# omuses/hqp

Hardware: AMD Instinct MI355X
Metric: KKT factor+solve/sec (fp64) (higher is better)
Workload: dtype f64; 1 GPU; C4 = BASELINE configs[3], the metric's 10^6-variable DOCP: multistage LQ optimal control QP, K=200 stages, nx=5000 states, nu=50 controls -> n=1015000 me=1005000 m=20000, dense fx/fu handed over as blocks, x_0 fixed, box bounds on u; plugin LQDOCP (STAGED engine), one system per GPU; stages=200, nx=5000, nu=50, n=1015000, me=1005000, m=20000, plugin=LQDOCP, kkt_dim_full=2040000

## Files before the change

__graft_entry__.py:

```python
from __future__ import annotations

import os
import subprocess
import sys

ROOT = os.path.dirname(os.path.abspath(__file__))
if ROOT not in sys.path:
    sys.path.insert(0, ROOT)

CSRC = os.path.join(ROOT, "hqp_amd", "csrc")
LIB = os.path.join(ROOT, "hqp_amd", "libhqpkkt.so")
LIB_RCCL = os.path.join(ROOT, "hqp_amd", "libhqpkkt_rccl.so")
HIPCC = os.environ.get("HIPCC", "/opt/rocm/bin/hipcc")


def _stale(target, sources):
    if not os.path.exists(target):
        return True
    t = os.path.getmtime(target)
    return any(os.path.getmtime(s) > t for s in sources)


def build(force=False):
    units = ("hqpkkt.hip", "tree.hip", "staged_engine.hip", "ip_loops.hip", "analysis.cpp", "staged_plan.cpp")
    srcs = [os.path.join(CSRC, f) for f in units + ("hqpkkt_handle.hpp", "device_common.hip.h", "analysis.hpp", "kernels.hip.h",
                                                    "ipdriver.hip.h", "factor_blk.hip.h", "solve_top.hip.h", "staged.hip.h", "staged_gemm.hip.h", "staged_sparse.hip.h", "staged_profile.hip.h", "staged_rows.hip.h",
                                                    "staged_host.hip.h", "staged_plan.hpp", "sk_table.hpp", "gemm_form.hpp")]
    srcs.append(os.path.join(ROOT, "include", "hqpkkt.h"))
    if force or _stale(LIB, srcs):
        cmd = [HIPCC, "--offload-arch=gfx950", "-O3", "-std=c++17", "-fPIC", "-shared",
               "-Wall", "-Wno-unused-function", "-o", LIB] + [os.path.join(CSRC, f) for f in units]
        subprocess.check_call(cmd, cwd=ROOT)
    rsrc = [os.path.join(CSRC, "rccl_exchange.cpp"), os.path.join(ROOT, "include", "hqpkkt_rccl.h")]
    if force or _stale(LIB_RCCL, rsrc):
        subprocess.check_call([HIPCC, "--offload-arch=gfx950", "-O2", "-std=c++17", "-fPIC", "-shared", "-Wall",
                               "-o", LIB_RCCL, rsrc[0], "-ldl"], cwd=ROOT)
    subprocess.check_call(["make", "-s", "-C", os.path.join(ROOT, "oracle"), "all"])
    import hqp_amd
    from hqp_amd import _lib
    L = _lib.lib()
    for sym in _lib.SYMBOLS:
# ... 50 lines not shown
```

hqp_amd/_lib.py:

```python
from __future__ import annotations

import ctypes as C
import os

import numpy as np

_HERE = os.path.dirname(os.path.abspath(__file__))
LIB_PATH = os.environ.get("HQPKKT_LIB") or os.path.join(_HERE, "libhqpkkt.so")

OK, E_SIZES, E_MEM, E_SING, E_FORMAT, E_NULL, E_RANGE, E_INTERN, E_DEVICE = 0, 1, 3, 4, 6, 8, 10, 17, 100
MODE_FULL, MODE_REDUCED, MODE_STAGED = 0, 1, 2
LOC_HOST, LOC_DEVICE = 0, 1
DYN_DENSE, DYN_SPARSE, DYN_PROFILE = 0, 1, 3

SYMBOLS = [
    "hqpkkt_default_opts", "hqpkkt_create", "hqpkkt_destroy", "hqpkkt_analyze",
    "hqpkkt_set_values", "hqpkkt_factor", "hqpkkt_step", "hqpkkt_residual", "hqpkkt_solve",
    "hqpkkt_get_sbw", "hqpkkt_get_perm", "hqpkkt_set_tol", "hqpkkt_set_eps",
    "hqpkkt_set_stream", "hqpkkt_get_stats", "hqpkkt_strerror", "hqpkkt_debug_get",
    "hqpkkt_selftest_mfma", "hqpkkt_set_profile", "hqpkkt_get_profile",
    "hqpkkt_profile_class_name", "hqpkkt_set_shard", "hqpkkt_debug_read",
    "hqpkkt_default_ip_opts", "hqpkkt_mehrotra", "hqpkkt_franke",
    "hqpkkt_set_stages", "hqpkkt_debug_stage_ranks", "hqpkkt_debug_stage_block", "hqpkkt_debug_dgemm", "hqpkkt_debug_dgemm2", "hqpkkt_debug_dgemm_full", "hqpkkt_debug_sk_table", "hqpkkt_debug_gemm_form",
    "hqpkkt_analyze_staged", "hqpkkt_set_values_staged", "hqpkkt_set_shard_stream",
    "hqpkkt_values_staging", "hqpkkt_detect_stages", "hqpkkt_stage_staging", "hqpkkt_set_stage_block",
    "hqpkkt_debug_factor_block", "hqpkkt_debug_solve_top_stamps", "hqpkkt_set_dynamics_form", "hqpkkt_set_dense_columns",
    "hqpkkt_debug_sk_profile", "hqpkkt_debug_gemv_profile",
    "hqpkkt_set_packed_panels", "hqpkkt_debug_dgemm_packed", "hqpkkt_debug_gemv_packed", "hqpkkt_debug_carried_packed",
    "hqpkkt_set_dense_rows",
]
RCCL_LIB_PATH = os.path.join(_HERE, "libhqpkkt_rccl.so")
RCCL_SYMBOLS = ["hqpkkt_rccl_unique_id", "hqpkkt_rccl_create", "hqpkkt_rccl_create_from_env",
                "hqpkkt_rccl_comm_info", "hqpkkt_rccl_exchange", "hqpkkt_rccl_destroy", "hqpkkt_rccl_origin"]

XCHG_ALLGATHER, XCHG_ALLREDUCE_SUM, XCHG_BCAST_BASE = 0, 1, 16
EXCHANGE_FN = C.CFUNCTYPE(C.c_int, C.c_void_p, C.c_int, C.c_void_p, C.c_longlong, C.c_int)


class Opts(C.Structure):
    _fields_ = [("mode", C.c_int), ("device", C.c_int), ("loc", C.c_int), ("tol", C.c_double),
                ("eps", C.c_double), ("pivot_eps", C.c_double), ("leaf_size", C.c_int),
                ("max_pivots", C.c_int), ("zd_policy", C.c_int), ("slack_policy", C.c_int),
                ("no_small_fronts", C.c_int), ("upd_pingpong_mb", C.c_int), ("amalgamation", C.c_int),
                ("ordering", C.c_int)]
# ... 102 lines not shown
    L.hqpkkt_set_values_staged.argtypes = [vp, dp, vp, vp, dp, dp]
    L.hqpkkt_values_staging.argtypes = [vp, C.POINTER(C.c_void_p), C.POINTER(C.c_void_p), C.POINTER(C.c_void_p)]
    L.hqpkkt_set_shard_stream.argtypes = [vp, C.c_int, C.c_int, vp, vp]
    L.hqpkkt_debug_dgemm.argtypes = [C.c_int] * 7 + [C.POINTER(C.c_double)] * 2
    L.hqpkkt_debug_stage_block.argtypes = [vp, C.c_int, vp, C.c_longlong, C.POINTER(C.c_longlong)]
    L.hqpkkt_debug_dgemm2.argtypes = [C.c_int] * 8 + [C.POINTER(C.c_double)] * 2 + [C.POINTER(C.c_longlong)]
    L.hqpkkt_debug_dgemm_full.argtypes = [C.c_int, C.POINTER(DgemmCase)]
    L.hqpkkt_debug_sk_table.argtypes = [C.c_longlong, C.c_int, C.c_int, C.c_int, C.POINTER(C.c_int), C.c_longlong, C.POINTER(C.c_longlong),
                                        C.POINTER(C.c_int), C.POINTER(C.c_int)]
    L.hqpkkt_debug_sk_profile.argtypes = [C.POINTER(C.c_int), C.c_longlong, C.c_int, C.POINTER(C.c_int), C.c_longlong, C.POINTER(C.c_longlong)]
    L.hqpkkt_debug_gemv_profile.argtypes = [C.c_int] * 4 + [vp, C.c_longlong, C.c_longlong, vp, vp, vp, C.c_double, vp]
    L.hqpkkt_debug_dgemm_packed.argtypes = [C.c_int, C.POINTER(DgemmCase), vp, C.c_longlong, vp]
    L.hqpkkt_debug_gemv_packed.argtypes = [C.c_int] * 4 + [vp, C.c_longlong, vp, vp, vp, vp, C.c_double, vp]
    L.hqpkkt_debug_carried_packed.argtypes = [C.c_int] * 4 + [vp, C.c_longlong, C.c_longlong, vp, C.c_longlong, vp, vp, vp] + [C.c_longlong] * 4
    L.hqpkkt_debug_gemm_form.argtypes = [C.c_int] * 7 + [C.c_longlong] * 3 + [C.c_int, C.POINTER(C.c_longlong)] + [C.POINTER(C.c_int)] * 3
    L.hqpkkt_debug_solve_top_stamps.argtypes = [vp, vp, C.c_int]
    L.hqpkkt_debug_factor_block.argtypes = [C.c_int, C.c_int, vp, C.c_double, C.c_double, C.c_int, C.c_int] + [vp] * 7
    _lib = L
    return L


_rccl = None


def rccl_lib():
    global _rccl
    if _rccl is None:
        lib()
        R = C.CDLL(RCCL_LIB_PATH)
        R.hqpkkt_rccl_unique_id.argtypes = [C.c_char_p]
# ... 12 lines not shown
```

hqp_amd/csrc/hqpkkt.hip:

```cpp
#include "hqpkkt_handle.hpp"

char g_last_hip_error[512] = "";
std::atomic<long long> g_live_bufs[2];

namespace kktdev {
__global__ void k_mfma_selftest(const double *A, const double *B, double *C) {
  const int lane = threadIdx.x & 63, lr = lane & 15, lk = lane >> 4;
  double4_t acc = {0.0, 0.0, 0.0, 0.0};
  for (int k0 = 0; k0 < 16; k0 += 4)
    acc = mfma_f64(A[lr * 16 + k0 + lk], B[(k0 + lk) * 16 + lr], acc);
  for (int rg = 0; rg < 4; rg++) C[(lk + 4 * rg) * 16 + lr] = acc[rg];
}
}

int hqpkkt_default_opts(hqpkkt_opts *o) {
  if (!o) return HQPKKT_E_NULL;
  std::memset(o, 0, sizeof(*o));
  o->mode = HQPKKT_MODE_FULL;
  o->device = 0;
  o->loc = HQPKKT_LOC_HOST;
  o->tol = 1.0;
  o->eps = 1e-10;
  o->pivot_eps = 1e-20;
  o->leaf_size = 0;
// ... 621 lines not shown
    case 0: v = &an.q2e; break;
    case 1: v = &an.piv_start; break;
    case 2: v = &an.npiv; break;
    case 3: v = &an.nbor; break;
    case 4: v = &an.parent; break;
    case 5: v = &an.level; break;
    case 6:
      tmp.assign(an.bptr.begin(), an.bptr.end());
      v = &tmp;
      break;
    case 7: v = &an.bidx; break;
    case 8: v = &an.ent_er; break;
    case 9: v = &an.ent_ec; break;
    case 10: v = &an.node_owner; break;
    case 11: v = &an.xroots; break;
    case 20: case 21: case 22: case 23: case 24: case 25: case 26: case 27: case 28: case 32: case 33: case 34: case 35: case 36: case 37: case 38: case 39: case 41: case 42: case 43: {
      const int e = staged_debug_get(h, what, tmp);
      if (e) return e;
      v = &tmp;
      break;
    }
    case 30:
      tmp = {h->zd_used, h->zd_weak ? 1 : 0};
      v = &tmp;
      break;
    case 31:
      tmp = {h->top_n, h->top_n ? h->top_lt : h->an.nlevels, (int)h->top_lds, h->top_ns, h->small_tree ? 1 : 0, h->tree_factor ? 1 : 0, h->top_split ? 1 : 0};
      v = &tmp;
      break;
    case 40:
      tmp = {(int)g_live_bufs[0].load(), (int)g_live_bufs[1].load()};
// ... 79 lines not shown
```

hqp_amd/csrc/staged.hip.h:

```cpp
#pragma once
#include <hip/hip_runtime.h>

#include <algorithm>

#include "staged_plan.hpp"
#include "staged_gemm.hip.h"

namespace stg {

struct HTerm {
  int s1, s2, wi;
};
__global__ void k_st_add_h(int nent, const long long *__restrict__ dst, const int *__restrict__ tptr,
                           const HTerm *__restrict__ terms, const double *__restrict__ vals,
                           const double *__restrict__ wt, double *__restrict__ G, int add) {
  const int e = blockIdx.x * blockDim.x + threadIdx.x;
  if (e >= nent) return;
  double s = 0.0;
  for (int k = tptr[e]; k < tptr[e + 1]; k++) s += vals[terms[k].s1] * vals[terms[k].s2] * wt[terms[k].wi];
  if (add)
    G[dst[e]] += s;
  else
    G[dst[e]] = s;
}
// ... 1900 lines not shown
```

hqp_amd/csrc/staged_engine.hip:

```cpp
#include "hqpkkt_handle.hpp"

#include <algorithm>

#include "staged.hip.h"
#include "staged_sparse.hip.h"
#include "staged_profile.hip.h"
#include "staged_rows.hip.h"
#include "staged_host.hip.h"

int staged_dense_products(hqpkkt_t *h, const Vecs &v, const double **x1, const double **x2, int *ndyn) {
  StagedDev &d = *h->sd;
  const kktdev::StagedPlan &P = d.plan;
  if (!P.dense_dyn) return 0;
  int nzmax = 1, npmax = 1;
  for (int k = 0; k < P.K; k++) nzmax = std::max(nzmax, P.nk[k] + P.mk[k]), npmax = std::max(npmax, P.nk[k + 1]);
  nzmax = std::max(nzmax, P.nk[P.K]);
  if (P.sharded) {
    const long long tot = d.dyn_sum_x2 + P.ndyn;
    KLAUNCH(h, KC_RESIDUAL, stg::k_st_zero<<<nblk(tot), 256, 0, h->stream>>>(tot, d.dyn_sum.p));
    KLAUNCH(h, KC_RESIDUAL, stg::k_st_dynloc_ax<<<dim3(std::min((npmax + 3) / 4, 2048), P.K), 256, 0, h->stream>>>(d.dyn_loc.p, d.F.p, v.dx,
                                                                                                           d.dyn_sum.p + d.dyn_sum_x2));
    KLAUNCH(h, KC_RESIDUAL, stg::k_st_dynloc_aty<<<dim3((nzmax + 255) / 256, P.K + 1), 256, 0, h->stream>>>(d.dyn_loc.p, d.F.p, v.dy, d.dyn_sum.p));
    int e = exchange(h, HQPKKT_XCHG_ALLREDUCE_SUM, d.dyn_sum.p, tot, 1);
    if (e) return e;
// ... 96 lines not shown
      out = P.pf_ptr;
      for (size_t q = 0; q < P.pf_rng.size() / 2; q++)
        out.push_back(P.packed ? (int)P.pk_off[q] : -1), out.push_back(P.packed ? P.pk_ld[q] : 0);
      break;
    case 43:
      if (P.rows_min > 0) {
        out = P.wr_ptr;
        out.insert(out.end(), P.wr_rows.begin(), P.wr_rows.end());
        for (int k = 0; k <= P.K; k++)
          for (long long c : {P.h_kept[k], P.h_cut[k]}) out.push_back((int)(unsigned)(c & 0xffffffffLL)), out.push_back((int)(c >> 32));
      }
      break;
    case 38:
      for (const StagedDev::SkTab &t : h->sd->sk_tabs)
        for (int val : {(int)t.tiles, (int)t.nslab, t.form, t.list, t.hits}) out.push_back(val);
      break;
    default: return HQPKKT_E_RANGE;
  }
  return 0;
}

extern "C" {

int hqpkkt_set_dynamics_form(hqpkkt_t *h, int form) {
  return guarded([&]() -> int {
    if (!h) return HQPKKT_E_NULL;
    if (h->opts.mode != HQPKKT_MODE_STAGED) return HQPKKT_E_INTERN;
    if (form != HQPKKT_DYN_DENSE && form != HQPKKT_DYN_SPARSE && form != HQPKKT_DYN_PROFILE) return HQPKKT_E_RANGE;
    if (!h->sd) h->sd.reset(new StagedDev);
    h->sd->plan.want_sparse = form == HQPKKT_DYN_SPARSE;
// ... 487 lines not shown
  return 0;
}
int hqpkkt_debug_dgemm(int device, int M, int N, int K, int lower, int mirror, int reps, double *ms, double *max_err) {
  return debug_dgemm(device, M, N, K, 0, lower, mirror, reps, ms, max_err, nullptr);
}
int hqpkkt_debug_dgemm2(int device, int M, int N, int K, int K2, int lower, int mirror, int reps, double *ms, double *max_err, long long *asym) {
  return debug_dgemm(device, M, N, K, K2, lower, mirror, reps, ms, max_err, asym);
}
int hqpkkt_debug_dgemm_full(int device, hqpkkt_dgemm_case *c) {
  return guarded([&]() -> int { return debug_dgemm_full(device, c); });
}
int hqpkkt_debug_dgemm_packed(int device, hqpkkt_dgemm_case *c, const double *packed, long long packed_elems, const long long *panel) {
  return guarded([&]() -> int { return packed ? debug_dgemm_full(device, c, packed, packed_elems, panel) : HQPKKT_E_NULL; });
}

int hqpkkt_debug_gemm_form(int M, int N, int K, int lower, int mirror, int cus, int grid, long long sk_tiles, long long ws_elems,
                           long long ws2_elems, int flags, long long *tiles, int *table, int *tile_map, int *nsplit) {
  const stg::GemmForm f = stg::gemm_form(M, N, K, lower, mirror, cus, grid, sk_tiles, ws_elems, ws2_elems, flags);
  if (tiles) *tiles = f.tiles;
  if (table) *table = f.kind == stg::GEMM_FORM_CUT;
  if (tile_map) *tile_map = f.tile_map;
  if (nsplit) *nsplit = f.nsplit;
  return f.kind;
}

int hqpkkt_debug_sk_table(long long tiles, int nslab, int grid, int kind, int *units, long long cap_ints, long long *pieces, int *whole_a, int *whole_b) {
  stg::SplitTable t;
  if (!stg::gemm_list_table(kind, tiles, nslab, grid, t)) return 0;
  if (pieces) *pieces = t.pieces;
  if (whole_a) *whole_a = t.nA;
// ... 124 lines not shown
```

hqp_amd/csrc/staged_host.hip.h:

```cpp
#pragma once

struct StagedDev {
  kktdev::StagedPlan plan;
  DBuf<double> F, V, misc;
  DBuf<int> dyn, eq_rows, fix_rows, fix_src, h_tptr, chk_idx, chk_kind;
  DBuf<long long> h_dst, a_dst;
  DBuf<long long> c_dst;
  DBuf<int> wr_rows;
  DBuf<stg::HTerm> h_terms;
  DBuf<stg::DynDesc> dyn_desc;
  DBuf<double> dyn_x1, dyn_x2;
  DBuf<int> sp_arow, sp_tcol;
  DBuf<int> sp_tcol_light, hv_cols, hv_of;
  DBuf<double> dyn_part;
  int dyn_part_cols = 0;
  PinnedBuf<double> hblk[2];
  EventOwner hblk_ev[2];
  std::vector<char> blocks_set;
  DBuf<stg::StripTab> wtabs;
  DBuf<stg::RectTab> rtabs;
  DBuf<int> gtile;
  DBuf<unsigned> gowned;
  std::vector<long long> gowned_off;
  DBuf<stg::PackRect> prects;
// ... 31 lines not shown
      if (e.first == T) return e.second.p;
    if (!create) return nullptr;
    const std::vector<int> m = stg::gemm_tri_order(T);
    DBuf<int> b;
    if (b.upload(m)) return nullptr;
    tri_maps.emplace_back(T, std::move(b));
    return tri_maps.back().second.p;
  }
  struct SkTab {
    long long tiles, nslab;
    int form, list, stride, hits;
    DBuf<stg::SkUnit> units;
  };
  std::vector<SkTab> sk_tabs;
  bool sk_tables_on = true;
  SkTab *sk_tab(long long tiles, long long nslab, int form) {
    for (auto &e : sk_tabs)
      if (e.tiles == tiles && e.nslab == nslab && e.form == form) return &e;
    return nullptr;
  }
  stg::GemmForm gemm_form(int M, int N, int K, int lower, int mirror, bool first_stream = true) const {
    return stg::gemm_form(M, N, K, lower, mirror, cus, sk_grid, sk_tiles, sk_ws_elems, ks_ws2_elems,
                          (plan.sharded ? stg::GEMM_SHARDED : 0) | (first_stream ? 0 : stg::GEMM_SECOND_STREAM));
  }
  int sk_tab_prepare(const stg::GemmForm &f, long long nslab) {
    if (sk_tab(f.tiles, nslab, f.kind)) return 0;
    stg::SplitTable t;
    SkTab e{f.tiles, nslab, f.kind, 0, 0, 0, {}};
    e.list = stg::gemm_choose_list(f.kind == stg::GEMM_FORM_FRAC, sk_tables_on && !plan.sharded, f.tiles, nslab, sk_grid, sk_tiles, sk_ws_elems, t);
    if (e.list != stg::SK_LIST_NONE) {
// ... 131 lines not shown
    if (f.tile_map && !d.tri_map(T, true)) return HQPKKT_E_MEM;
    std::vector<int> order;
    if (f.tile_map) order = stg::gemm_tri_order(T);
    return d.pf_tab_prepare(f, g.M, g.N, g.lower, by, f.tile_map ? order.data() : nullptr, panel, npanel);
  }
  if (f.tile_map && !(g.tile_map = d.tri_map((g.M + 127) / 128))) return HQPKKT_E_INTERN;
  if (d.zeros.p && stg::gemm_operands_dma_ok(g)) g.zeros = d.zeros.p;
  if (P.pk_stage(k)) (by == 2 ? g.apack : g.bpack) = d.pk_tab.p + P.pf_ptr[k];
  StagedDev::PfTab *tab = d.pf_tab(g.M, g.N, g.lower, by, panel, npanel);
  if (!tab) return HQPKKT_E_INTERN;
  tab->hits++;
  const stg::SplitPlan sk{d.sk_ws.p, d.sk_cnt.p, tab->units.p, tab->stride};
  const stg::GemmLaunch L{stg::gemm_variant_for(g, d.gemm_variant), d.cus, d.sk_grid, &sk, nullptr};
  stg::gemm_launch_form(f, L, h->stream, g, [&](auto &&launch) { KLAUNCH(h, cls, launch()); });
  return 0;
}

int st_gemv_rows(hqpkkt_t *h, stg::GemvRows g) {
  if (g.M <= 0) return 0;
  KLAUNCH(h, KC_ST_VEC, stg::k_st_gemv_rows<<<(g.M + 3) / 4, 256, 0, h->stream>>>(g));
  return 0;
}
bool symv_tiles_form(const stg::GemvRows &g) {
  return !(env_no_symv() || g.M != g.N || g.N < env_symv_from() || (g.lda & 1) || (((size_t)g.A) & 15));
}
long long symv_tiles(int N) {
  const int nrt = (N + stg::SV_R - 1) / stg::SV_R;
  long long tiles = 0;
  for (int bi = 0; bi < nrt; bi++) tiles += bi / (stg::SV_C / stg::SV_R) + 1;
  return tiles;
// ... 509 lines not shown
      }
    }
    d.gowned_off[P.K] = (long long)ow.size();
    if (ow.empty()) ow.push_back(0u);
    if ((e = d.wtabs.upload(wt)) || (e = d.rtabs.upload(rt)) || (e = d.prects.upload(pr)) || (e = d.gtile.upload(gt)) ||
        (e = d.gowned.upload(ow)))
      return e;
    if (!d.ev_x1) HIPCHK(hipEventCreateWithFlags(&d.ev_x1.h, hipEventDisableTiming));
    if (h->xchg_sfn && !d.stream_x) {
      HIPCHK(hipStreamCreateWithFlags(&d.stream_x.h, hipStreamNonBlocking));
      for (EventOwner *ev : {&d.ev_w[0], &d.ev_w[1], &d.ev_w[2], &d.ev_x[0], &d.ev_x[1], &d.ev_x[2]})
        HIPCHK(hipEventCreateWithFlags(&ev->h, hipEventDisableTiming));
    }
  }
  d.sk_tables_on = stg::gemm_sk_table_from_env();
  d.sk_tabs.clear();
  d.pf_tabs.clear(), d.pf_rng.release(), d.pf_part.release(), d.pk_tab.release(), d.pk_part.release();
  if (P.profile_dyn && !P.pf_rng.empty()) {
    long long part = 1;
    for (int k = 0; k < P.K; k++)
      if (P.pf_stage[k])
        part = std::max(part, (long long)stg::pf_chunks(P.pf_rng.data() + 2 * (size_t)P.pf_ptr[k], P.panels(k), P.nk[k + 1]) * (P.nk[k] + P.mk[k]));
    if ((e = d.pf_rng.upload(P.pf_rng)) || (e = d.pf_part.alloc((size_t)part))) return e;
    if (P.packed) {
      std::vector<stg::PackPanel> tab(P.pk_off.size(), stg::PackPanel{0, 0});
      long long cpart = 1;
      for (int k = 0; k < P.K; k++) {
        if (!P.pk_stage(k)) continue;
        for (int q = P.pf_ptr[k]; q < P.pf_ptr[k + 1]; q++) tab[q] = stg::PackPanel{P.pk_off[q] - 16LL * P.pf_rng[2 * q] * P.pk_ld[q], P.pk_ld[q]};
        cpart = std::max(cpart, (long long)stg::pk_chunks(P.pf_rng.data() + 2 * (size_t)P.pf_ptr[k], P.panels(k), P.nk[k + 1]) * P.cap[k + 1] * (P.nk[k] + P.mk[k]));
// ... 242 lines not shown
  if (!ovl) {
    if ((e = st_gemm(h, stg::GemmArgs{sp.F, ldf, W, ldf, nullptr, 0, G, ldg, nz, nz, np, 1.0, 0.0, 1, 0}))) return e;
    st_add_h(h, d, P.h_ptr[k], ne_x + ne_u, G);
    if ((e = st_add_h_wide(h, d, k, G, ldg))) return e;
  } else {
    if ((e = st_gemm(h, stg::GemmArgs{sp.F, ldf, W, ldf, nullptr, 0, G, ldg, nn, nn, np, 1.0, 0.0, 1, 0}))) return e;
    st_add_h(h, d, P.h_ptr[k], ne_x, G);
    h->stream = sB;
    if ((e = st_gemm(h, stg::GemmArgs{W + nn, ldf, sp.F, ldf, nullptr, 0, G + nn * ldg, ldg, mm, nz, np, 1.0, 0.0, 0, 0}, KC_ST_GEMM, false))) return e;
    st_add_h(h, d, P.h_mid[k], ne_u, G);
  }
  h->stream = sB;
  if ((e = st_carried_rows(h, d, k, sp, sn, !ovl)) || (e = st_eliminate(h, d, k, sp, sn, G, !ovl))) return e;
  h->stream = sA;
  if ((e = chain.join())) return e;
  return st_gemm(h, stg::GemmArgs{sp.Y, P.ldy[k], sp.Rm, P.ldy[k], G, ldg, sp.V, P.ldv[k], nn, nn, P.qmax[k], -1.0, 1.0, 1, 1}, KC_ST_GEMM_UPD);
}

static int staged_stage_profile(hqpkkt_t *h, int k) {
  StagedDev &d = *h->sd;
  const kktdev::StagedPlan &P = d.plan;
  StagePtr sp = stage_ptr(d, k), sn = stage_ptr(d, k + 1);
  const int nn = P.nk[k], mm = P.mk[k], np = P.nk[k + 1], nz = nn + mm;
  const long long ldf = P.ldf[k], ldg = P.ldg[k], ldvn = P.ldv[k + 1];
  double *G = d.misc.p + P.oG, *W = d.misc.p + P.oW;
  int e;
  if ((e = st_gemm_profile(h, stg::GemmArgs{sn.V, ldvn, sp.F, ldf, nullptr, 0, W, ldf, np, nz, np, 1.0, 0.0, 0, 0}, k, 1)) ||
      (e = st_gemm_profile(h, stg::GemmArgs{sp.F, ldf, W, ldf, nullptr, 0, G, ldg, nz, nz, np, 1.0, 0.0, 1, 0}, k, 2)))
    return e;
  st_add_h(h, d, P.h_ptr[k], P.h_ptr[k + 1] - P.h_ptr[k], G);
  if ((e = st_add_h_wide(h, d, k, G, ldg))) return e;
  if (P.pk_stage(k)) {
    const int ek = P.eq_ptr[k + 1] - P.eq_ptr[k];
    stg::pk_launch_carried(stg::PkCarried{sn.BT, P.ldb[k + 1], sp.F, d.pk_tab.p + P.pf_ptr[k], d.pf_rng.p + 2 * (size_t)P.pf_ptr[k], np, nz, P.cap[k + 1], 0,
                                          sp.N + (size_t)ek * P.ldn[k], P.ldn[k], d.pk_part.p},
                           P.pf_rng.data() + 2 * (size_t)P.pf_ptr[k], h->stream, [&](auto &&launch) { KLAUNCH(h, KC_ST_GEMM_UPD, launch()); });
  } else if ((e = st_carried_rows(h, d, k, sp, sn, true)))
    return e;
  if ((e = st_eliminate(h, d, k, sp, sn, G, true))) return e;
  return st_gemm(h, stg::GemmArgs{sp.Y, P.ldy[k], sp.Rm, P.ldy[k], G, ldg, sp.V, P.ldv[k], nn, nn, P.qmax[k], -1.0, 1.0, 1, 1}, KC_ST_GEMM_UPD);
}

static stg::SpCols sp_cols(hqpkkt_t *h, StagedDev &d, int k, int c0, int ncols, bool light = false) {
  const kktdev::StagedPlan &P = d.plan;
  const int *ent = light && P.heavy_count(k) ? d.sp_tcol_light.p : d.sp_tcol.p;
  return stg::SpCols{ent + 2 * ((long long)P.nmk[k] + c0), h->td.AT.col.p, h->td.AT.val.p, P.nks[k], ncols};
}
static int staged_stage_sparse(hqpkkt_t *h, int k) {
  StagedDev &d = *h->sd;
  const kktdev::StagedPlan &P = d.plan;
  StagePtr sp = stage_ptr(d, k), sn = stage_ptr(d, k + 1);
  const int nn = P.nk[k], mm = P.mk[k], np = P.nk[k + 1], nz = nn + mm;
  const int ek = P.eq_ptr[k + 1] - P.eq_ptr[k], cx = P.cap[k + 1];
  const long long ldt = P.ldv[k + 1], ldg = P.ldg[k];
  double *G = d.misc.p + P.oG, *T = d.misc.p + P.oW;
// ... 15 lines not shown
                                 stg::SpGather{f, T, ldt, nz, G, ldg, G, ldg, 1}));
  }
  if (cx > 0 && nz > 0)
    KLAUNCH(h, KC_ST_SPARSE, stg::k_sp_carried<<<dim3(cb, (cx + 7) / 8), 256, 0, h->stream>>>(
                                 stg::SpCarried{f, sn.BT, P.ldb[k + 1], cx, sp.N + (size_t)ek * P.ldn[k], P.ldn[k]}));
  if (nd > 0) {
    KLAUNCH(h, KC_ST_SPARSE, stg::k_sp_gather<<<dim3(cb, (nd + stg::SP_RB - 1) / stg::SP_RB), 256, 0, h->stream>>>(
                                 stg::SpGather{f, Th, ldt, nd, Gh, ldg, nullptr, 0, 0}));
    if ((e = st_gemm(h, stg::GemmArgs{D, ldd, Wh, ldd, nullptr, 0, Ghh, ldd, nd, nd, np, 1.0, 0.0, 0, 0}))) return e;
    if (cx > 0 && (e = st_gemm(h, stg::GemmArgs{sn.BT, P.ldb[k + 1], D, ldd, nullptr, 0, Nh, ldd, cx, nd, np, 1.0, 0.0, 0, 0}, KC_ST_GEMM_UPD))) return e;
    KLAUNCH(h, KC_ST_SPARSE, stg::k_sp_heavy_place<<<dim3((unsigned)((std::max(nz, cx) + 255) / 256), nd), 256, 0, h->stream>>>(stg::SpHeavyPlace{
                                 nz, nd, cx, d.hv_cols.p + P.hv_ptr[k], d.hv_of.p + P.nmk[k], Gh, ldg, Ghh, ldd, G, ldg, Nh, sp.N + (size_t)ek * P.ldn[k], P.ldn[k]}));
  }
  st_add_h(h, d, P.h_ptr[k], P.h_ptr[k + 1] - P.h_ptr[k], G);
  if ((e = st_add_h_wide(h, d, k, G, ldg)) || (e = st_eliminate(h, d, k, sp, sn, G, true))) return e;
  return st_gemm(h, stg::GemmArgs{sp.Y, P.ldy[k], sp.Rm, P.ldy[k], G, P.ldg[k], sp.V, P.ldv[k], nn, nn, P.qmax[k], -1.0, 1.0, 1, 1}, KC_ST_GEMM_UPD);
}

static int staged_run_factor(hqpkkt_t *h, const double *z, const double *w) {
  Analysis &an = h->an;
  StagedDev &d = *h->sd;
  kktdev::StagedPlan &P = d.plan;
  hipStream_t s = h->stream;
  const int m = an.m, K = P.K;
  const bool timed = !h->capturing && !h->listing;
  int e;
  if (!h->listing) {
    const long long vk = (long long)P.nk[K] * P.ldv[K];
    kktdev::k_clear<<<(int)std::max<long long>(1, std::min<long long>(4096, (vk / 2 + 1023) / 1024)), 256, 0, s>>>(stage_ptr(d, K).V, vk, h->td.flags.p);
  }
  if (timed) HIPCHK(hipEventRecord(h->ev0, s));
  if (m > 0) KLAUNCH(h, KC_ASSEMBLE, k_weights<<<nblk(m), 256, 0, s>>>(1, m, an.n + an.me, z, w, h->td.wt.p, nullptr, h->td.flags.p));
  if (timed) HIPCHK(hipEventRecord(h->ev1, s));
  {
    StagePtr sp = stage_ptr(d, K);
    const int nK = P.nk[K], eK = P.eq_ptr[K + 1] - P.eq_ptr[K];
    st_add_h(h, d, P.h_ptr[K], P.h_ptr[K + 1] - P.h_ptr[K], sp.V, 0);
    if (!P.sharded && (e = st_add_h_wide(h, d, K, sp.V, P.ldv[K]))) return e;
    KLAUNCH(h, KC_ST_SMALL, stg::k_st_last<<<nblk(std::max(nK, 1)), 256, 0, s>>>(nK, eK, P.cap[K], sp.N, P.ldn[K], sp.BT, P.ldb[K], sp.dyn));
    if (P.sharded) st_keep_rows(h, d, K);
  }
// ... 163 lines not shown
```

hqp_amd/ipmatrix.py:

```python
from __future__ import annotations

import ctypes as C

import numpy as np

from . import _lib


class KktError(RuntimeError):
    def __init__(self, code, where):
        super().__init__(f"hqpkkt status {code} in {where}: {_lib.strerror(code)}")
        self.code = code


class SingularError(KktError):
    """E_SING of the reference (meschach/err.h:88)."""


def _check(code, where):
    if code == _lib.OK:
        return
    if code == _lib.E_SING:
        raise SingularError(code, where)
    raise KktError(code, where)
# ... 478 lines not shown
    return y


def carried_packed(BT, R, packed, panel, ranges, K, N, C_buf, c_row0, c_col0, device=0):
    import numpy as np
    pk, pan = _packed_args(packed, panel)
    r = np.ascontiguousarray(ranges, dtype=np.int32)
    for a in (BT, C_buf):
        assert a.dtype == np.float64 and a.ndim == 2 and a.flags.c_contiguous
    assert r.size == 2 * ((N + 127) // 128) == pan.size
    _check(_lib.lib().hqpkkt_debug_carried_packed(device, K, N, R, BT.ctypes.data, BT.shape[0], BT.shape[1], pk.ctypes.data, pk.size, pan.ctypes.data,
                                                  r.ctypes.data, C_buf.ctypes.data, C_buf.shape[0], C_buf.shape[1], c_row0, c_col0), "debug_carried_packed")
    return C_buf


SK_KINDS = ("unequal", "equal", "frac")


def sk_table(tiles, nslab, grid=512, kind="unequal"):
    import numpy as np
    k = SK_KINDS.index(kind)
    pieces, wa, wb = C.c_longlong(), C.c_int(), C.c_int()
    stride = _lib.lib().hqpkkt_debug_sk_table(tiles, nslab, grid, k, None, 0, C.byref(pieces), C.byref(wa), C.byref(wb))
    if stride <= 0:
        return None
    u = np.zeros((grid, stride, 6), dtype=np.int32)
    got = _lib.lib().hqpkkt_debug_sk_table(tiles, nslab, grid, k, u.ctypes.data_as(C.POINTER(C.c_int)), u.size, C.byref(pieces), C.byref(wa), C.byref(wb))
    assert got == stride
    return u, pieces.value, wa.value, wb.value

# ... 45 lines not shown
```

include/hqpkkt.h:

```cpp
#ifndef HQPKKT_H
#define HQPKKT_H

#ifdef __cplusplus
extern "C" {
#endif

#define HQPKKT_VERSION 1

#define HQPKKT_OK 0
#define HQPKKT_E_SIZES 1
#define HQPKKT_E_MEM 3
#define HQPKKT_E_SING 4
#define HQPKKT_E_FORMAT 6
#define HQPKKT_E_NULL 8
#define HQPKKT_E_RANGE 10
#define HQPKKT_E_INTERN 17
#define HQPKKT_E_DEVICE 100

#define HQPKKT_MODE_FULL 0
#define HQPKKT_MODE_REDUCED 1
#define HQPKKT_MODE_STAGED 2

#define HQPKKT_LOC_HOST 0
#define HQPKKT_LOC_DEVICE 1
// ... 120 lines not shown
} hqpkkt_dgemm_operand;
typedef struct hqpkkt_dgemm_case {
  int M, N, K, K2;
  int lower, mirror, flags, cin_is_c;
  double alpha, beta;
  hqpkkt_dgemm_operand A, B, A2, B2, Cin;
  double *C;
  long long c_rows, ldc, c_row0, c_col0;
  int form, tile_map, ldsdma, nsplit;
  long long tiles;
  const int *krange;
  int krange_by;
} hqpkkt_dgemm_case;
int hqpkkt_debug_dgemm_full(int device, hqpkkt_dgemm_case *c);

int hqpkkt_debug_sk_table(long long tiles, int nslab, int grid, int kind, int *units, long long cap_ints, long long *pieces, int *whole_a, int *whole_b);

int hqpkkt_debug_sk_profile(const int *ranges, long long tiles, int grid, int *units, long long cap_ints, long long *pieces);

int hqpkkt_debug_gemv_profile(int device, int rows_form, int K, int N, const double *A, long long a_rows, long long ld, const int *ranges,
                              const double *x, const double *add, double alpha, double *y);

int hqpkkt_debug_dgemm_packed(int device, hqpkkt_dgemm_case *c, const double *packed, long long packed_elems, const long long *panel);
int hqpkkt_debug_gemv_packed(int device, int rows_form, int K, int N, const double *packed, long long packed_elems, const long long *panel,
                             const int *ranges, const double *x, const double *add, double alpha, double *y);
int hqpkkt_debug_carried_packed(int device, int K, int N, int R, const double *BT, long long bt_rows, long long ldb, const double *packed,
                                long long packed_elems, const long long *panel, const int *ranges, double *C, long long c_rows, long long ldc,
                                long long c_row0, long long c_col0);

int hqpkkt_debug_gemm_form(int M, int N, int K, int lower, int mirror, int cus, int grid, long long sk_tiles, long long ws_elems,
// ... 49 lines not shown
```

Before: 0.8360 KKT factor+solve/s.

## Add streaming symmetric low-rank update kernel for staged V = G - Y^T Rm

Adds a dedicated kernel for the per-stage update V = G - Y^T·Rm when the inner dimension q is at most 64. It walks only lower-triangular 64x64 tiles, computes the product with f64 MFMA, subtracts from G in one pass and writes both the tile and its transpose through LDS. This replaces the generic GEMM path for this call, which is meant to save its setup and its separate read-modify-write traffic on a memory-bound rank-q update. The old product path is kept for sharded runs, misaligned or odd sizes, and when an environment variable forces it; debug entry points and counters are added alongside.

```diff
diff --git a/__graft_entry__.py b/__graft_entry__.py
--- a/__graft_entry__.py
+++ b/__graft_entry__.py
@@ -24,7 +24,7 @@
 def build(force=False):
     units = ("hqpkkt.hip", "tree.hip", "staged_engine.hip", "ip_loops.hip", "analysis.cpp", "staged_plan.cpp")
     srcs = [os.path.join(CSRC, f) for f in units + ("hqpkkt_handle.hpp", "device_common.hip.h", "analysis.hpp", "kernels.hip.h",
-                                                    "ipdriver.hip.h", "factor_blk.hip.h", "solve_top.hip.h", "staged.hip.h", "staged_gemm.hip.h", "staged_sparse.hip.h", "staged_profile.hip.h", "staged_rows.hip.h",
+                                                    "ipdriver.hip.h", "factor_blk.hip.h", "solve_top.hip.h", "staged.hip.h", "staged_gemm.hip.h", "staged_update.hip.h", "update_form.hpp", "staged_sparse.hip.h", "staged_profile.hip.h", "staged_rows.hip.h",
                                                     "staged_host.hip.h", "staged_plan.hpp", "sk_table.hpp", "gemm_form.hpp")]
     srcs.append(os.path.join(ROOT, "include", "hqpkkt.h"))
     if force or _stale(LIB, srcs):
diff --git a/hqp_amd/_lib.py b/hqp_amd/_lib.py
--- a/hqp_amd/_lib.py
+++ b/hqp_amd/_lib.py
@@ -28,6 +28,7 @@
     "hqpkkt_debug_sk_profile", "hqpkkt_debug_gemv_profile",
     "hqpkkt_set_packed_panels", "hqpkkt_debug_dgemm_packed", "hqpkkt_debug_gemv_packed", "hqpkkt_debug_carried_packed",
     "hqpkkt_set_dense_rows",
+    "hqpkkt_debug_update_v", "hqpkkt_debug_update_form",
 ]
 RCCL_LIB_PATH = os.path.join(_HERE, "libhqpkkt_rccl.so")
 RCCL_SYMBOLS = ["hqpkkt_rccl_unique_id", "hqpkkt_rccl_create", "hqpkkt_rccl_create_from_env",
@@ -160,6 +161,9 @@
     L.hqpkkt_debug_gemv_packed.argtypes = [C.c_int] * 4 + [vp, C.c_longlong, vp, vp, vp, vp, C.c_double, vp]
     L.hqpkkt_debug_carried_packed.argtypes = [C.c_int] * 4 + [vp, C.c_longlong, C.c_longlong, vp, C.c_longlong, vp, vp, vp] + [C.c_longlong] * 4
     L.hqpkkt_debug_gemm_form.argtypes = [C.c_int] * 7 + [C.c_longlong] * 3 + [C.c_int, C.POINTER(C.c_longlong)] + [C.POINTER(C.c_int)] * 3
+    L.hqpkkt_debug_update_v.argtypes = ([C.c_int] * 3 + [vp, C.c_longlong, vp, C.c_longlong, C.c_longlong, C.c_longlong] + [vp] + [C.c_longlong] * 4
+                                        + [vp] + [C.c_longlong] * 4 + [C.POINTER(C.c_int)])
+    L.hqpkkt_debug_update_form.argtypes = [C.c_int] * 4 + [C.c_longlong] * 3 + [C.c_ulonglong] * 4
     L.hqpkkt_debug_solve_top_stamps.argtypes = [vp, vp, C.c_int]
     L.hqpkkt_debug_factor_block.argtypes = [C.c_int, C.c_int, vp, C.c_double, C.c_double, C.c_int, C.c_int] + [vp] * 7
     _lib = L
diff --git a/hqp_amd/csrc/hqpkkt.hip b/hqp_amd/csrc/hqpkkt.hip
--- a/hqp_amd/csrc/hqpkkt.hip
+++ b/hqp_amd/csrc/hqpkkt.hip
@@ -659,7 +659,7 @@
     case 9: v = &an.ent_ec; break;
     case 10: v = &an.node_owner; break;
     case 11: v = &an.xroots; break;
-    case 20: case 21: case 22: case 23: case 24: case 25: case 26: case 27: case 28: case 32: case 33: case 34: case 35: case 36: case 37: case 38: case 39: case 41: case 42: case 43: {
+    case 20: case 21: case 22: case 23: case 24: case 25: case 26: case 27: case 28: case 32: case 33: case 34: case 35: case 36: case 37: case 38: case 39: case 41: case 42: case 43: case 44: {
       const int e = staged_debug_get(h, what, tmp);
       if (e) return e;
       v = &tmp;
diff --git a/hqp_amd/csrc/staged.hip.h b/hqp_amd/csrc/staged.hip.h
--- a/hqp_amd/csrc/staged.hip.h
+++ b/hqp_amd/csrc/staged.hip.h
@@ -5,6 +5,7 @@
 
 #include "staged_plan.hpp"
 #include "staged_gemm.hip.h"
+#include "staged_update.hip.h"
 
 namespace stg {
 
diff --git a/hqp_amd/csrc/staged_engine.hip b/hqp_amd/csrc/staged_engine.hip
--- a/hqp_amd/csrc/staged_engine.hip
+++ b/hqp_amd/csrc/staged_engine.hip
@@ -134,6 +134,9 @@
     case 38:
       for (const StagedDev::SkTab &t : h->sd->sk_tabs)
         for (int val : {(int)t.tiles, (int)t.nslab, t.form, t.list, t.hits}) out.push_back(val);
+      break;
+    case 44:
+      out = {h->sd->upd_streamed, h->sd->upd_product};
       break;
     default: return HQPKKT_E_RANGE;
   }
@@ -651,6 +654,54 @@
   return guarded([&]() -> int { return packed ? debug_dgemm_full(device, c, packed, packed_elems, panel) : HQPKKT_E_NULL; });
 }
 
+static int debug_update_v(int device, int nn, int q, const double *Y, long long y_col0, const double *Rm, long long rm_col0, long long yr_rows,
+                          long long ldy, const double *G, long long g_rows, long long ldg, long long g_row0, long long g_col0, double *V,
+                          long long v_rows, long long ldv, long long v_row0, long long v_col0, int *path) {
+  if (!Y || !Rm || !G || !V) return HQPKKT_E_NULL;
+  if (nn <= 0 || q < 0) return HQPKKT_E_RANGE;
+  if (ldy < 1 || y_col0 < 0 || rm_col0 < 0 || y_col0 + nn > ldy || rm_col0 + nn > ldy || yr_rows < (long long)q + 1) return HQPKKT_E_RANGE;
+  if (ldg < 1 || g_row0 < 0 || g_col0 < 0 || g_col0 + nn > ldg || g_row0 + nn > g_rows) return HQPKKT_E_RANGE;
+  if (ldv < 1 || v_row0 < 0 || v_col0 < 0 || v_col0 + nn > ldv || v_row0 + nn > v_rows) return HQPKKT_E_RANGE;
+  int ndev = 0;
+  if (hipGetDeviceCount(&ndev) != hipSuccess || ndev <= device) return HQPKKT_E_DEVICE;
+  HIPCHK(hipSetDevice(device));
+  DBuf<double> dY, dR, dG, dV;
+  auto up = [](DBuf<double> &d, const double *p, long long elems) -> int {
+    if (d.alloc((size_t)elems)) return HQPKKT_E_MEM;
+    HIPCHK(hipMemcpy(d.p, p, sizeof(double) * (size_t)elems, hipMemcpyHostToDevice));
+    return 0;
+  };
+  int e;
+  if ((e = up(dY, Y, yr_rows * ldy)) || (e = up(dR, Rm, yr_rows * ldy)) || (e = up(dG, G, g_rows * ldg)) || (e = up(dV, V, v_rows * ldv))) return e;
+  const double *pY = dY.p + y_col0, *pR = dR.p + rm_col0, *pG = dG.p + g_row0 * ldg + g_col0;
+  double *pV = dV.p + v_row0 * ldv + v_col0;
+  const char *env = getenv("HQPKKT_UPDATE_PRODUCT");
+  const bool streams = stg::update_v_streams(false, env && atoi(env) != 0, q, nn, ldg, ldv, ldy, (uintptr_t)pG, (uintptr_t)pV, (uintptr_t)pY, (uintptr_t)pR);
+  if (streams)
+    stg::update_v_launch(stg::UpdateV{pY, pR, ldy, pG, ldg, pV, ldv, nn, q}, 0);
+  else {
+    stg::GemmArgs g{pY, ldy, pR, ldy, pG, ldg, pV, ldv, nn, nn, q, -1.0, 1.0, 1, 1};
+    DebugGemm run;
+    if ((e = run.prepare(device, g, 0))) return e;
+    run.launch(g);
+  }
+  HIPCHK(hipDeviceSynchronize());
+  HIPCHK(hipMemcpy(V, dV.p, sizeof(double) * (size_t)(v_rows * ldv), hipMemcpyDeviceToHost));
+  if (path) *path = streams ? 1 : 0;
+  return 0;
+}
+int hqpkkt_debug_update_v(int device, int nn, int q, const double *Y, long long y_col0, const double *Rm, long long rm_col0, long long yr_rows,
+                          long long ldy, const double *G, long long g_rows, long long ldg, long long g_row0, long long g_col0, double *V,
+                          long long v_rows, long long ldv, long long v_row0, long long v_col0, int *path) {
+  return guarded([&]() -> int {
+    return debug_update_v(device, nn, q, Y, y_col0, Rm, rm_col0, yr_rows, ldy, G, g_rows, ldg, g_row0, g_col0, V, v_rows, ldv, v_row0, v_col0, path);
+  });
+}
+int hqpkkt_debug_update_form(int sharded, int force_product, int q, int nn, long long ldg, long long ldv, long long ldy, unsigned long long g,
+                             unsigned long long v, unsigned long long y, unsigned long long rm) {
+  return stg::update_v_streams(sharded != 0, force_product != 0, q, nn, ldg, ldv, ldy, (uintptr_t)g, (uintptr_t)v, (uintptr_t)y, (uintptr_t)rm) ? 1 : 0;
+}
+
 int hqpkkt_debug_gemm_form(int M, int N, int K, int lower, int mirror, int cus, int grid, long long sk_tiles, long long ws_elems,
                            long long ws2_elems, int flags, long long *tiles, int *table, int *tile_map, int *nsplit) {
   const stg::GemmForm f = stg::gemm_form(M, N, K, lower, mirror, cus, grid, sk_tiles, ws_elems, ws2_elems, flags);
diff --git a/hqp_amd/csrc/staged_host.hip.h b/hqp_amd/csrc/staged_host.hip.h
--- a/hqp_amd/csrc/staged_host.hip.h
+++ b/hqp_amd/csrc/staged_host.hip.h
@@ -69,6 +69,8 @@
   };
   std::vector<SkTab> sk_tabs;
   bool sk_tables_on = true;
+  bool update_product = false;
+  int upd_streamed = 0, upd_product = 0;
   SkTab *sk_tab(long long tiles, long long nslab, int form) {
     for (auto &e : sk_tabs)
       if (e.tiles == tiles && e.nslab == nslab && e.form == form) return &e;
@@ -230,6 +232,20 @@
   const stg::GemmLaunch L{stg::gemm_variant_for(g, d.gemm_variant), d.cus, d.sk_grid, &sk, nullptr};
   stg::gemm_launch_form(f, L, h->stream, g, [&](auto &&launch) { KLAUNCH(h, cls, launch()); });
   return 0;
+}
+
+int st_update_v(hqpkkt_t *h, StagedDev &d, int k, const StagePtr &sp, const double *G) {
+  const kktdev::StagedPlan &P = d.plan;
+  const int nn = P.nk[k], q = P.qmax[k];
+  if (nn <= 0) return 0;
+  if (stg::update_v_streams(P.sharded, d.update_product, q, nn, P.ldg[k], P.ldv[k], P.ldy[k], (uintptr_t)G, (uintptr_t)sp.V, (uintptr_t)sp.Y,
+                            (uintptr_t)sp.Rm)) {
+    d.upd_streamed++;
+    KLAUNCH(h, KC_ST_GEMM_UPD, stg::update_v_launch(stg::UpdateV{sp.Y, sp.Rm, P.ldy[k], G, P.ldg[k], sp.V, P.ldv[k], nn, q}, h->stream));
+    return 0;
+  }
+  d.upd_product++;
+  return st_gemm(h, stg::GemmArgs{sp.Y, P.ldy[k], sp.Rm, P.ldy[k], G, P.ldg[k], sp.V, P.ldv[k], nn, nn, q, -1.0, 1.0, 1, 1}, KC_ST_GEMM_UPD);
 }
 
 int st_gemv_rows(hqpkkt_t *h, stg::GemvRows g) {
@@ -769,6 +785,7 @@
     }
   }
   d.sk_tables_on = stg::gemm_sk_table_from_env();
+  d.update_product = getenv("HQPKKT_UPDATE_PRODUCT") && atoi(getenv("HQPKKT_UPDATE_PRODUCT")) != 0;
   d.sk_tabs.clear();
   d.pf_tabs.clear(), d.pf_rng.release(), d.pf_part.release(), d.pk_tab.release(), d.pk_part.release();
   if (P.profile_dyn && !P.pf_rng.empty()) {
@@ -1041,7 +1058,7 @@
   if ((e = st_carried_rows(h, d, k, sp, sn, !ovl)) || (e = st_eliminate(h, d, k, sp, sn, G, !ovl))) return e;
   h->stream = sA;
   if ((e = chain.join())) return e;
-  return st_gemm(h, stg::GemmArgs{sp.Y, P.ldy[k], sp.Rm, P.ldy[k], G, ldg, sp.V, P.ldv[k], nn, nn, P.qmax[k], -1.0, 1.0, 1, 1}, KC_ST_GEMM_UPD);
+  return st_update_v(h, d, k, sp, G);
 }
 
 static int staged_stage_profile(hqpkkt_t *h, int k) {
@@ -1065,7 +1082,7 @@
   } else if ((e = st_carried_rows(h, d, k, sp, sn, true)))
     return e;
   if ((e = st_eliminate(h, d, k, sp, sn, G, true))) return e;
-  return st_gemm(h, stg::GemmArgs{sp.Y, P.ldy[k], sp.Rm, P.ldy[k], G, ldg, sp.V, P.ldv[k], nn, nn, P.qmax[k], -1.0, 1.0, 1, 1}, KC_ST_GEMM_UPD);
+  return st_update_v(h, d, k, sp, G);
 }
 
 static stg::SpCols sp_cols(hqpkkt_t *h, StagedDev &d, int k, int c0, int ncols, bool light = false) {
@@ -1111,7 +1128,7 @@
   }
   st_add_h(h, d, P.h_ptr[k], P.h_ptr[k + 1] - P.h_ptr[k], G);
   if ((e = st_add_h_wide(h, d, k, G, ldg)) || (e = st_eliminate(h, d, k, sp, sn, G, true))) return e;
-  return st_gemm(h, stg::GemmArgs{sp.Y, P.ldy[k], sp.Rm, P.ldy[k], G, P.ldg[k], sp.V, P.ldv[k], nn, nn, P.qmax[k], -1.0, 1.0, 1, 1}, KC_ST_GEMM_UPD);
+  return st_update_v(h, d, k, sp, G);
 }
 
 static int staged_run_factor(hqpkkt_t *h, const double *z, const double *w) {
@@ -1122,6 +1139,7 @@
   const int m = an.m, K = P.K;
   const bool timed = !h->capturing && !h->listing;
   int e;
+  d.upd_streamed = d.upd_product = 0;
   if (!h->listing) {
     const long long vk = (long long)P.nk[K] * P.ldv[K];
     kktdev::k_clear<<<(int)std::max<long long>(1, std::min<long long>(4096, (vk / 2 + 1023) / 1024)), 256, 0, s>>>(stage_ptr(d, K).V, vk, h->td.flags.p);
diff --git a/hqp_amd/csrc/staged_update.hip.h b/hqp_amd/csrc/staged_update.hip.h
--- /dev/null
+++ b/hqp_amd/csrc/staged_update.hip.h
@@ -0,0 +1,140 @@
+#pragma once
+#include <hip/hip_runtime.h>
+
+#include "update_form.hpp"
+
+namespace stg {
+
+struct UpdateV {
+  const double *Y, *Rm;
+  long long ldy;
+  const double *G;
+  long long ldg;
+  double *V;
+  long long ldv;
+  int nn, q;
+};
+
+template <int NCH>
+__global__ void __launch_bounds__(256, 4) k_st_update_v(UpdateV u) {
+  constexpr int T = UPD_T, KC = UPD_KC, LDT = T + 1;
+  static_assert(T == 64 && KC == 32, "the thread maps below are written for 64 x 64 tiles and 256 threads");
+  __shared__ __attribute__((aligned(16))) double lds[T * LDT];
+  double *As = lds, *Bs = lds + KC * T;
+  const int tid = threadIdx.x, lane = tid & 63, wave = tid >> 6;
+  const int t = xcd_swizzle(blockIdx.x, gridDim.x);
+  int tm = (int)((sqrtf(8.0f * (float)t + 1.0f) - 1.0f) * 0.5f);
+  while ((tm + 1) * (tm + 2) / 2 <= t) tm++;
+  while (tm * (tm + 1) / 2 > t) tm--;
+  const int tn = t - tm * (tm + 1) / 2;
+  const int i0 = tm * T, j0 = tn * T;
+  const bool diag = tm == tn;
+  const int cp = 2 * (tid & 31), r8 = tid >> 5;
+  const bool ain = i0 + cp < u.nn, bin = j0 + cp < u.nn;
+  const long long acol = ain ? i0 + cp : 0, bcol = bin ? j0 + cp : 0;
+  double2_t pa[4], pb[4];
+  auto request = [&](int c) {
+#pragma unroll
+    for (int p = 0; p < 4; p++) {
+      const int k = c * KC + 8 * p + r8, kc = k < u.q ? k : u.q - 1;
+      pa[p] = *(const double2_t *)(u.Y + (long long)kc * u.ldy + acol);
+      pb[p] = *(const double2_t *)(u.Rm + (long long)kc * u.ldy + bcol);
+    }
+  };
+  request(0);
+  __builtin_amdgcn_sched_barrier(0);
+  double2_t g[8];
+#pragma unroll
+  for (int p = 0; p < 8; p++) {
+    const int i = i0 + 8 * p + r8, ic = i < u.nn ? i : u.nn - 1;
+    g[p] = *(const double2_t *)(u.G + (long long)ic * u.ldg + bcol);
+  }
+  __builtin_amdgcn_sched_barrier(0);
+  const int wm = wave >> 1, wn = wave & 1, lr = lane & 15, lk = lane >> 4;
+  double4_t acc[2][2];
+#pragma unroll
+  for (int x = 0; x < 2; x++)
+#pragma unroll
+    for (int y = 0; y < 2; y++) acc[x][y] = (double4_t){0.0, 0.0, 0.0, 0.0};
+  const int nks = 4 * ((u.q + 15) / 16);
+#pragma unroll
+  for (int c = 0; c < NCH; c++) {
+    if (c > 0) __syncthreads();
+#pragma unroll
+    for (int p = 0; p < 4; p++) {
+      const int kr = 8 * p + r8;
+      const bool live = c * KC + kr < u.q;
+      const double2_t zero = (double2_t){0.0, 0.0};
+      *(double2_t *)(As + kr * T + cp) = live && ain ? pa[p] : zero;
+      *(double2_t *)(Bs + kr * T + cp) = live && bin ? pb[p] : zero;
+    }
+    if (c + 1 < NCH) request(c + 1);
+    __syncthreads();
+    const double *Ab = As + wm * 32 + lr, *Bb = Bs + wn * 32 + lr;
+    auto steps = [&](int ks0) {
+#pragma unroll
+      for (int ks = ks0; ks < ks0 + 4; ks++) {
+        double af[2], bf[2];
+#pragma unroll
+        for (int x = 0; x < 2; x++) af[x] = Ab[(ks * 4 + lk) * T + 16 * x];
+#pragma unroll
+        for (int y = 0; y < 2; y++) bf[y] = Bb[(ks * 4 + lk) * T + 16 * y];
+#pragma unroll
+        for (int x = 0; x < 2; x++)
+#pragma unroll
+          for (int y = 0; y < 2; y++) acc[x][y] = mfma_f64(af[x], bf[y], acc[x][y]);
+      }
+    };
+    steps(0);
+    if (nks - 8 * c > 4) steps(4);
+  }
+  __syncthreads();
+  auto fresh = [](int x) {
+    asm volatile("" : "+v"(x));
+    return x;
+  };
+  const int cq = fresh(cp), rq = fresh(r8);
+#pragma unroll
+  for (int x = 0; x < 2; x++)
+#pragma unroll
+    for (int y = 0; y < 2; y++)
+#pragma unroll
+      for (int rg = 0; rg < 4; rg++) lds[(wm * 32 + 16 * x + lk + 4 * rg) * LDT + wn * 32 + 16 * y + lr] = acc[x][y][rg];
+  __syncthreads();
+  double2_t v[8];
+#pragma unroll
+  for (int p = 0; p < 8; p++) {
+    const int r = 8 * p + rq;
+    v[p].x = g[p].x - lds[r * LDT + cq];
+    v[p].y = g[p].y - lds[r * LDT + cq + 1];
+    if (!diag && i0 + r < u.nn && bin) *(double2_t *)(u.V + (long long)(i0 + r) * u.ldv + j0 + cq) = v[p];
+  }
+  __syncthreads();
+#pragma unroll
+  for (int p = 0; p < 8; p++) {
+    const int r = 8 * p + rq;
+    lds[cq * LDT + r] = v[p].x;
+    lds[(cq + 1) * LDT + r] = v[p].y;
+  }
+  __syncthreads();
+#pragma unroll
+  for (int p = 0; p < 8; p++) {
+    const int r = 8 * p + rq;
+    const double2_t w = (double2_t){lds[r * LDT + cq], lds[r * LDT + cq + 1]};
+    if (!ain) continue;
+    if (diag) {
+      if (i0 + r < u.nn)
+        *(double2_t *)(u.V + (long long)(i0 + r) * u.ldv + i0 + cq) = (double2_t){cq <= r ? v[p].x : w.x, cq + 1 <= r ? v[p].y : w.y};
+    } else if (j0 + r < u.nn)
+      *(double2_t *)(u.V + (long long)(j0 + r) * u.ldv + i0 + cq) = w;
+  }
+}
+
+static inline void update_v_launch(const UpdateV &u, hipStream_t s) {
+  const unsigned tiles = (unsigned)update_v_tiles(u.nn);
+  if (update_v_chunks(u.q) == 1)
+    k_st_update_v<1><<<tiles, 256, 0, s>>>(u);
+  else
+    k_st_update_v<2><<<tiles, 256, 0, s>>>(u);
+}
+}
diff --git a/hqp_amd/csrc/update_form.hpp b/hqp_amd/csrc/update_form.hpp
--- /dev/null
+++ b/hqp_amd/csrc/update_form.hpp
@@ -0,0 +1,22 @@
+#pragma once
+#include <cstdint>
+
+namespace stg {
+
+static const int UPD_T = 64;
+static const int UPD_QMAX = 64;
+
+static inline bool update_v_streams(bool sharded, bool force_product, int q, int nn, long long ldg, long long ldv, long long ldy,
+                                    uintptr_t g, uintptr_t v, uintptr_t y, uintptr_t rm) {
+  if (sharded || force_product) return false;
+  if (q < 1 || q > UPD_QMAX || nn < 2 || (nn & 1)) return false;
+  if (((ldg | ldv | ldy) & 1) || ldg < nn || ldv < nn || ldy < nn) return false;
+  return ((g | v | y | rm) & 15) == 0;
+}
+static const int UPD_KC = 32;
+static inline int update_v_chunks(int q) { return q <= UPD_KC ? 1 : 2; }
+static inline long long update_v_tiles(int nn) {
+  const long long t = (nn + UPD_T - 1) / UPD_T;
+  return t * (t + 1) / 2;
+}
+}
diff --git a/hqp_amd/ipmatrix.py b/hqp_amd/ipmatrix.py
--- a/hqp_amd/ipmatrix.py
+++ b/hqp_amd/ipmatrix.py
@@ -516,6 +516,22 @@
     return C_buf
 
 
+def update_v(Y, Rm, G, V_buf, nn, q, y_col0=0, rm_col0=0, g_row0=0, g_col0=0, v_row0=0, v_col0=0, device=0):
+    import numpy as np
+    for a in (Y, Rm, G, V_buf):
+        assert a.dtype == np.float64 and a.ndim == 2 and a.flags.c_contiguous
+    assert Y.shape == Rm.shape and V_buf.flags.writeable
+    path = C.c_int(-1)
+    _check(_lib.lib().hqpkkt_debug_update_v(device, nn, q, Y.ctypes.data, y_col0, Rm.ctypes.data, rm_col0, Y.shape[0], Y.shape[1],
+                                            G.ctypes.data, G.shape[0], G.shape[1], g_row0, g_col0,
+                                            V_buf.ctypes.data, V_buf.shape[0], V_buf.shape[1], v_row0, v_col0, C.byref(path)), "debug_update_v")
+    return ("product", "stream")[path.value]
+
+
+def update_form(q, nn, ldg, ldv, ldy, g=0, v=0, y=0, rm=0, sharded=False, force_product=False):
+    return bool(_lib.lib().hqpkkt_debug_update_form(int(sharded), int(force_product), q, nn, ldg, ldv, ldy, g, v, y, rm))
+
+
 SK_KINDS = ("unequal", "equal", "frac")
 
 
diff --git a/include/hqpkkt.h b/include/hqpkkt.h
--- a/include/hqpkkt.h
+++ b/include/hqpkkt.h
@@ -158,6 +158,12 @@
 } hqpkkt_dgemm_case;
 int hqpkkt_debug_dgemm_full(int device, hqpkkt_dgemm_case *c);
 
+int hqpkkt_debug_update_v(int device, int nn, int q, const double *Y, long long y_col0, const double *Rm, long long rm_col0, long long yr_rows,
+                          long long ldy, const double *G, long long g_rows, long long ldg, long long g_row0, long long g_col0, double *V,
+                          long long v_rows, long long ldv, long long v_row0, long long v_col0, int *path);
+int hqpkkt_debug_update_form(int sharded, int force_product, int q, int nn, long long ldg, long long ldv, long long ldy, unsigned long long g,
+                             unsigned long long v, unsigned long long y, unsigned long long rm);
+
 int hqpkkt_debug_sk_table(long long tiles, int nslab, int grid, int kind, int *units, long long cap_ints, long long *pieces, int *whole_a, int *whole_b);
 
 int hqpkkt_debug_sk_profile(const int *ranges, long long tiles, int grid, int *units, long long cap_ints, long long *pieces);
```

Result: no change. 0.8433 KKT factor+solve/s, median of 6 (+0.9%).
